# cvlab-dresden/DSAC

Measured on AMD Instinct MI355X. Metric: hypotheses scored/sec over 640x480 coord map, higher is better.
Workload: dtype f32

## Files before the change

dsac_amd/csrc/k2_plan.h:

```cpp
#pragma once

namespace dk {

struct K2Opts {
    bool pixel_minor = true;
    int flags = 0;
    int variant = -1;
    bool exact_auto = true;
    int diag = 0;
    int f16_store = 1;
};
enum { K2_ELEM_F32 = 0, K2_ELEM_F16 = 1, K2_ELEM_BF16 = 2 };
constexpr int K2_FLAG_STORE_ONLY = 1 << 1;
constexpr int K2_FLAG_ERR_UNFUSED = 1 << 24;
constexpr int K2_FLAG_PRECISE = 1 << 25;
constexpr int K2_FLAG_REC32 = 1 << 26;
constexpr int K2_FLAG_RECLO = 1 << 27;
constexpr int K2_FLAG_EXACT = 1 << 28;
constexpr int K2_FLAG_EXACT_ANY = 1 << 29;
enum { K2_FORM_NONE = 0, K2_FORM_FP32_VALU = 1, K2_FORM_FP32_MFMA = 2, K2_FORM_RECLO = 3, K2_FORM_EXACT_VEC = 4, K2_FORM_EXACT_ANY = 5, K2_FORM_PRECISE = 6 };
enum { K2_WHY_AUTO_OFF = 1, K2_WHY_FORCED = 2, K2_WHY_FOCAL = 4, K2_WHY_NO_POSES = 8 };
constexpr int K2_NF_MULTIPLE = 128;
constexpr int K2_WG = 256;

inline bool k2_wants_exact(const K2Opts& o) {
    if (o.flags & (K2_FLAG_EXACT | K2_FLAG_EXACT_ANY)) return true;
    return o.exact_auto && o.variant < 0 && !(o.flags & (K2_FLAG_PRECISE | K2_FLAG_RECLO | K2_FLAG_STORE_ONLY | K2_FLAG_REC32));
}

enum { K2_EXONLY_OK = 0, K2_EXONLY_VARIANT = 1, K2_EXONLY_FLAGS = 2, K2_EXONLY_AUTO_OFF = 3 };
inline int k2_exact_only(int variant, int flags, bool exact_auto) {
    const int ex_bits = K2_FLAG_EXACT | K2_FLAG_EXACT_ANY;
    if (variant != -1) return K2_EXONLY_VARIANT;
    if (flags & ~ex_bits) return K2_EXONLY_FLAGS;
    if (!exact_auto && !(flags & ex_bits)) return K2_EXONLY_AUTO_OFF;
    return K2_EXONLY_OK;
}

constexpr double K2_BIG_BYTES = 1.0e9, K2_HUGE_BYTES = 4.4e9;
inline double k2_err_bytes(int N, int P) { return (double)N * (double)P * 4.0; }
constexpr int K2_SMALL_MAP_CELLS = 16384;

inline bool k2_fuse_sums(const K2Opts& o, int N, int P, bool want_err, bool want_soft) {
    return !want_soft && want_err && o.variant < 0 && !(o.flags & K2_FLAG_ERR_UNFUSED) && k2_err_bytes(N, P) > K2_BIG_BYTES;
}

#define K2_FP32_IDS(VA, HP, ST, PS)                                                                                                                         \
    VA(0, 4, 32, false) VA(1, 4, 32, true) VA(2, 4, 16, false) VA(3, 4, 64, false) VA(10, 4, 1, false) VA(11, 4, 2, false) VA(12, 4, 4, false)               \
    VA(13, 4, 8, false)                                                                                                                                     \
    HP(20, 64, 2) HP(21, 64, 4) HP(22, 128, 2) HP(23, 32, 2) HP(24, 64, 1) HP(25, 128, 4) HP(26, 32, 4) HP(27, 128, 1)                                         \
    ST(40, 1, 1, 4, false, 1) ST(41, 2, 1, 4, false, 1) ST(42, 4, 1, 4, false, 1) ST(43, 2, 2, 4, false, 1)                                                   \
    ST(44, 1, 4, 1, true, 1) ST(45, 2, 4, 1, true, 1) ST(46, 4, 4, 1, true, 1) ST(47, 1, 2, 1, true, 1) ST(48, 2, 2, 1, true, 1) ST(49, 4, 2, 1, true, 1)       \
    ST(50, 1, 1, 1, true, 1) ST(51, 2, 1, 1, true, 1) ST(52, 4, 1, 1, true, 1) ST(53, 2, 1, 4, true, 1) ST(54, 2, 2, 4, true, 1) ST(55, 4, 1, 4, true, 1)       \
    ST(56, 2, 4, 4, true, 1) ST(57, 4, 2, 4, true, 1) ST(58, 4, 4, 1, true, 4) ST(59, 2, 4, 1, true, 5)                                                       \
    PS(60, 1) PS(61, 2) PS(62, 4)                                                                                                                           \
    ST(65, 4, 4, 4, true, 4) ST(66, 4, 4, 2, true, 4) ST(67, 1, 4, 4, true, 1) ST(68, 2, 4, 4, false, 1) ST(69, 2, 4, 8, true, 1) ST(70, 2, 4, 4, true, 4)     \
    ST(71, 1, 4, 8, true, 1) ST(72, 2, 4, 16, true, 1) ST(73, 2, 8, 1, true, 1) ST(74, 1, 8, 1, true, 1) ST(75, 2, 6, 1, true, 1) ST(76, 2, 3, 1, true, 1)     \
    ST(77, 1, 6, 1, true, 1)                                                                                                                                \
    ST(80, 4, 4, 1, true, 4) ST(81, 4, 4, 1, true, 4) ST(82, 4, 4, 1, true, 4) ST(83, 4, 4, 1, true, 4) ST(84, 4, 4, 1, true, 4) ST(85, 4, 4, 1, true, 4)     \
    ST(89, 4, 4, 1, true, 4) ST(93, 4, 4, 1, true, 4) ST(94, 4, 4, 1, true, 4) ST(95, 4, 4, 1, true, 4)
#define K2_RECLO_IDS(LO) LO(80, 4, 4, 3) LO(81, 4, 4, 2) LO(82, 4, 2, 4) LO(83, 2, 4, 3)
constexpr int K2_RECLO_DEFAULT_ID = 81;
#define K2_EXACT_IDS(EX) EX(84, 4, 4, 2, 1) EX(85, 4, 4, 2, 2) EX(89, 2, 4, 2, 1) EX(93, 4, 1, 3, 1) EX(94, 4, 1, 3, 2) EX(95, 4, 1, 4, 2)
#define K2_EXACT_AUTO_TILES(AX) AX(4, 1, 3) AX(4, 4, 2)

enum { K2_FAM_NONE = 0, K2_FAM_VALU_SCALAR, K2_FAM_VALU, K2_FAM_HP, K2_FAM_ST, K2_FAM_PS, K2_FAM_RECLO, K2_FAM_EXACT_VEC, K2_FAM_EXACT_ANY, K2_FAM_PRECISE };

struct K2Kernel {
    int family = K2_FAM_NONE, id = -1;
    int px = 0, ht = 0, ng = 0, ch = 0, wv = 0, pw = 0, minw = 0, exf = 0;
};
inline K2Kernel k2_fp32_kernel(int id) {
    K2Kernel k;
    switch (id) {
#define K2_VA_(ID, PX, HT, SP) case ID: k.family = K2_FAM_VALU; k.id = ID; k.px = PX; k.ht = HT; break;
#define K2_HP_(ID, HT, CH) case ID: k.family = K2_FAM_HP; k.id = ID; k.ht = HT; k.ch = CH; break;
#define K2_ST_(ID, NG, CH, WV, PW, MW) case ID: k.family = K2_FAM_ST; k.id = ID; k.ng = NG; k.ch = CH; k.wv = WV; k.pw = PW; k.minw = MW; break;
#define K2_PS_(ID, NG) case ID: k.family = K2_FAM_PS; k.id = ID; k.ng = NG; k.wv = 4; break;
        K2_FP32_IDS(K2_VA_, K2_HP_, K2_ST_, K2_PS_)
#undef K2_VA_
#undef K2_HP_
#undef K2_ST_
#undef K2_PS_
        default: break;
    }
    return k;
}
inline K2Kernel k2_reclo_kernel(int id) {
    K2Kernel k;
    switch (id) {
#define K2_LO_(ID, NG, CH, MW) case ID: k.family = K2_FAM_RECLO; k.id = ID; k.ng = NG; k.ch = CH; k.wv = 1; k.pw = 1; k.minw = MW; break;
        K2_RECLO_IDS(K2_LO_)
#undef K2_LO_
        default: break;
    }
    return k;
}
inline K2Kernel k2_exact_kernel(int id) {
    K2Kernel k;
    switch (id) {
#define K2_EX_(ID, NG, CH, MW, F) case ID: k.family = K2_FAM_EXACT_VEC; k.id = ID; k.ng = NG; k.ch = CH; k.wv = 1; k.pw = 1; k.minw = MW; k.exf = F; break;
        K2_EXACT_IDS(K2_EX_)
#undef K2_EX_
        default: break;
    }
    return k;
}
inline bool k2_variant_known(int v) { return v == -1 || k2_fp32_kernel(v).family != K2_FAM_NONE; }

inline int reproject_num_pixel_tiles(int P) { return (P + 63) / 64 + 15; }
inline int k2_ceil_div(int a, int b) { return (a + b - 1) / b; }
inline int k2_tiles(const K2Kernel& k, int P, bool soft) {
    switch (k.family) {
        case K2_FAM_VALU_SCALAR: return k2_ceil_div(P, K2_WG);
        case K2_FAM_VALU: return k2_ceil_div(P, K2_WG * k.px);
        case K2_FAM_HP: return k2_ceil_div(P, K2_WG * k.ch);
        case K2_FAM_PS: return k2_ceil_div(P, 64);
        case K2_FAM_PRECISE: return 2 * k2_ceil_div(P, K2_WG * 4);
        case K2_FAM_ST: case K2_FAM_RECLO: case K2_FAM_EXACT_VEC: case K2_FAM_EXACT_ANY: {
            const int PT = k2_ceil_div(P, k.wv * k.ch * 64);
            const int rows = k.pw ? PT * k.wv : PT;
            return rows + ((k.family == K2_FAM_EXACT_ANY && (P & 3) != 0 && soft) ? 1 : 0);
        }
        default: return 0;
    }
}

struct K2PlanIn {
    K2Opts o;
    int N = 0, Nf = 0, frames = 1;
    int P = 0, W = 0;
    bool uv = false;
    bool xyz_al16 = true, uv_al16 = true, err_al16 = true;
    bool focal_ok = true;
    bool poses = true;
    bool want_err = false, want_soft = false;
    int err_elem = K2_ELEM_F32;
};
constexpr int K2_STATUS_OK = 0, K2_STATUS_INVALID = 1, K2_STATUS_NOT_SUPPORTED = 801;
struct K2Plan {
    int status = K2_STATUS_OK;
    int form = K2_FORM_NONE, why = 0;
    K2Kernel k;
    bool need_split = false, need_lo = false;
    bool fuse_sums = false;
    int kflags = 0;
    bool pixel_minor = true;
    int Nf = 0;
    int tiles = 0;
};

inline K2Plan k2_plan(const K2PlanIn& in) {
    K2Plan p;
    const K2Opts& o = in.o;
    const bool fuse = k2_fuse_sums(o, in.N, in.P, in.want_err, in.want_soft);
    const bool err = in.want_err, soft = in.want_soft || fuse;
    if (in.N <= 0 || in.P <= 0 || (!err && !soft)) return p;
    auto refuse = [](int status) { K2Plan r; r.status = status; return r; };
    if (in.Nf <= 0 || in.frames <= 1) p.Nf = ((in.N + 127) / 128) * 128;
    else if (in.Nf % K2_NF_MULTIPLE != 0) return refuse(K2_STATUS_INVALID);
    else p.Nf = in.Nf;
    p.fuse_sums = fuse;
    const int variant = o.variant;
    const bool vec = in.P % 4 == 0 && in.err_al16 && in.xyz_al16 && in.uv_al16;
    p.kflags = o.flags | ((variant >= 40 && !o.pixel_minor) ? 32 : 0);
    p.pixel_minor = o.pixel_minor;
    const bool split_ok = in.poses && k2_wants_exact(o) && in.focal_ok;
    const K2Kernel exk = k2_exact_kernel(variant), lok = k2_reclo_kernel(variant);
    const bool ex_variant = exk.family != K2_FAM_NONE;
    int why = 0;
    if (!(o.flags & (K2_FLAG_EXACT | K2_FLAG_EXACT_ANY))) {
        if (variant >= 0 || (o.flags & (K2_FLAG_PRECISE | K2_FLAG_RECLO | K2_FLAG_STORE_ONLY | K2_FLAG_REC32))) why |= K2_WHY_FORCED;
        else if (!o.exact_auto) why |= K2_WHY_AUTO_OFF;
    } else if (variant >= 0 && !ex_variant) why |= K2_WHY_FORCED;
    if (!in.focal_ok) why |= K2_WHY_FOCAL;
    if (!in.poses) why |= K2_WHY_NO_POSES;
    if (in.err_elem != K2_ELEM_F32 && !(err && vec && in.P % 8 == 0 && split_ok && k2_exact_only(variant, o.flags, o.exact_auto) == K2_EXONLY_OK))
        return refuse(K2_STATUS_NOT_SUPPORTED);
    const bool prec_map = vec && (in.uv || in.W % 4 == 0);
    if (in.poses && (((o.flags & K2_FLAG_PRECISE) && !prec_map) || ((o.flags & K2_FLAG_RECLO) && !vec) || ((o.flags & K2_FLAG_EXACT) && !(vec && split_ok)) ||
                     ((o.flags & K2_FLAG_EXACT_ANY) && !(split_ok && (variant < 0 || (ex_variant && vec))))))
        return refuse(K2_STATUS_NOT_SUPPORTED);
    if ((o.flags & K2_FLAG_EXACT_ANY) && !in.poses) return refuse(K2_STATUS_NOT_SUPPORTED);
    const bool small_map = in.P <= K2_SMALL_MAP_CELLS;
    if ((o.flags & K2_FLAG_PRECISE) && in.poses && prec_map) {
        p.form = K2_FORM_PRECISE;
        p.k.family = K2_FAM_PRECISE;
// ... 44 lines not shown
```

dsac_amd/csrc/k_forward.hip:

```cpp
#include "kernels.h"
#include <hip/hip_ext.h>
#include "dmath.h"

namespace dk {

typedef float f4 __attribute__((ext_vector_type(4)));
typedef float f2 __attribute__((ext_vector_type(2)));
typedef _Float16 h4 __attribute__((ext_vector_type(4)));

DM_INLINE void pose_focal(const float4* __restrict__ cams, int h, int Nf, float& fx, float& fy) {
    if (!cams) return;
    const float4 k = cams[Nf > 0 ? h / Nf : 0];
    fx = k.x; fy = k.y;
}
DM_INLINE int split_exponent_of(float fx, float fy) {
    int e = 0;
    while (e < 31 && (float)(1u << e) < fmaxf(fx, fy)) e++;
    return e;
}
__global__ __launch_bounds__(256) void k_pose_prep(int N, const double* __restrict__ poses, float fx, float fy, float* __restrict__ staged,
                                                   const float4* __restrict__ cams, int Nf) {
    const int h = blockIdx.x * blockDim.x + threadIdx.x;
    if (h >= N) return;
    pose_focal(cams, h, Nf, fx, fy);
// ... 455 lines not shown
    if (pt >= PT) return;
    const int h0 = ht * HT;
    const int nh = min(HT, N - h0);
    const int tid = threadIdx.x, lane = tid & 63, wave = tid >> 6;
    const int c = lane & 15, g = lane >> 4;
    {
        const int frame = h0 / Nf;
        xyz += (long long)frame * xyz_stride;
        if (UV) uv += (long long)frame * uv_stride;
    }

    __shared__ float s_A[(HT / 16) * 3 * 64];
    __shared__ float s_soft[SOFT ? (K2_THREADS / 64) * HT : 1];
    for (int i = tid; i < (HT / 16) * 3 * 64; i += K2_THREADS) {
        const int l = i & 63, cg = i >> 6;
        const int comp = cg % 3, gi = cg / 3;
        const int hyp = min(16 * gi + (l & 15), nh - 1), k = l >> 4;
        const float v = staged[(size_t)(h0 + hyp) * POSE_STRIDE + comp * 4 + k];
        s_A[i] = comp < 2 ? -v : v;
    }

    float Bm[KM_CH][4];
    f2 ppix[KM_CH][4];
    int p0[KM_CH];
    bool valid[KM_CH];
#pragma unroll
    for (int ch = 0; ch < KM_CH; ch++) {
        const int chunk0 = (pt * (K2_THREADS / 64) * KM_CH + wave * KM_CH + ch) * 64;
        p0[ch] = chunk0 + 4 * c;
        valid[ch] = p0[ch] < P;
#pragma unroll
        for (int m = 0; m < 4; m++) {
            const int pc = min(p0[ch] + m, P - 1);
            Bm[ch][m] = (g < 3) ? xyz[(size_t)pc * 3 + g] : 1.0f;
        }
        if (UV) {
            if (valid[ch]) {
                const f4* su = reinterpret_cast<const f4*>(uv + (size_t)p0[ch] * 2);
                const f4 u0 = su[0], u1 = su[1];
                ppix[ch][0] = f2{u0.x - cx, u0.y - cy}; ppix[ch][1] = f2{u0.z - cx, u0.w - cy};
                ppix[ch][2] = f2{u1.x - cx, u1.y - cy}; ppix[ch][3] = f2{u1.z - cx, u1.w - cy};
            } else {
                ppix[ch][0] = ppix[ch][1] = ppix[ch][2] = ppix[ch][3] = splat(0.f);
            }
        } else {
            int y = p0[ch] / W, x = p0[ch] - y * W;
#pragma unroll
            for (int m = 0; m < 4; m++) {
                ppix[ch][m] = f2{(float)x - cx, (float)y - cy};
                if (++x == W) { x = 0; y++; }
            }
        }
    }
    __syncthreads();

    for (int gi = 0; gi < HT / 16; gi++) {
        if (16 * gi >= nh) break;
        const float ax = s_A[(gi * 3 + 0) * 64 + lane], ay = s_A[(gi * 3 + 1) * 64 + lane], az = s_A[(gi * 3 + 2) * 64 + lane];
        const int hyp0 = 16 * gi + 4 * g;
        f2 ssum[4] = {splat(0.f), splat(0.f), splat(0.f), splat(0.f)};
#pragma unroll
        for (int ch = 0; ch < KM_CH; ch++) {
            f4 ev[4];
            f2 sloc[4];
            if (kflags & 2) {
                if (ERR && valid[ch]) {
                    f4* dst = reinterpret_cast<f4*>(err + (size_t)(h0 + hyp0) * P + p0[ch]);
                    const size_t rs = (size_t)P / 4;
                    const f4 o = {ax, ay, az, (float)gi};
#pragma unroll
                    for (int r = 0; r < 4; r++) {
                        if (hyp0 + r >= nh) continue;
                        f4* q = dst + r * rs;
                        const int mode = (kflags >> 2) & 7;
                        if (mode == 0) __builtin_nontemporal_store(o, q);
                        else if (mode == 1) *q = o;
                        else if (mode == 2) asm volatile("global_store_dwordx4 %0, %1, off sc1" ::"v"(q), "v"(o) : "memory");
                        else if (mode == 3) asm volatile("global_store_dwordx4 %0, %1, off sc0 sc1" ::"v"(q), "v"(o) : "memory");
                        else if (mode == 4) asm volatile("global_store_dwordx4 %0, %1, off sc1 nt" ::"v"(q), "v"(o) : "memory");
                        else asm volatile("global_store_dwordx4 %0, %1, off sc0" ::"v"(q), "v"(o) : "memory");
                    }
                }
                continue;
            }
            if (__builtin_expect(__any(hp_chunk<false, SOFT>(ax, ay, az, Bm[ch], ppix[ch], clampv, kA, kB, ev, sloc)), 0))
                (void)hp_chunk<true, SOFT>(ax, ay, az, Bm[ch], ppix[ch], clampv, kA, kB, ev, sloc);
            if (SOFT) {
                const f2 vf = splat(valid[ch] ? 1.0f : 0.0f);
#pragma unroll
                for (int r = 0; r < 4; r++) ssum[r] = pk_fma(sloc[r], vf, ssum[r]);
            }
            if (ERR && valid[ch]) {
                f4* dst = reinterpret_cast<f4*>(err + (size_t)(h0 + hyp0) * P + p0[ch]);
                const size_t rs = (size_t)P / 4;
                if (nh == HT) {
#pragma unroll
                    for (int r = 0; r < 4; r++) {
                        if (kflags & 1) dst[r * rs] = ev[r]; else __builtin_nontemporal_store(ev[r], dst + r * rs);
                    }
                } else {
#pragma unroll
                    for (int r = 0; r < 4; r++) {
                        if (hyp0 + r < nh) { if (kflags & 1) dst[r * rs] = ev[r]; else __builtin_nontemporal_store(ev[r], dst + r * rs); }
                    }
                }
            }
        }
        if (SOFT) {
            const float s0 = row16_sum(ssum[0].x + ssum[0].y), s1 = row16_sum(ssum[1].x + ssum[1].y);
            const float s2 = row16_sum(ssum[2].x + ssum[2].y), s3 = row16_sum(ssum[3].x + ssum[3].y);
            if (c == 0) {
                float* dst = s_soft + wave * HT + hyp0;
                if (hyp0 + 0 < nh) dst[0] = s0;
                if (hyp0 + 1 < nh) dst[1] = s1;
                if (hyp0 + 2 < nh) dst[2] = s2;
                if (hyp0 + 3 < nh) dst[3] = s3;
            }
        }
    }

    if (SOFT) {
        __syncthreads();
        if (tid < nh) {
            float s = 0.f;
#pragma unroll
            for (int w = 0; w < K2_THREADS / 64; w++) s += s_soft[w * HT + tid];
            soft_part[(size_t)pt * N + h0 + tid] = s;
        }
    }
}

template <int HT, int KM_CH>
static hipError_t launch_reproject_hp(hipStream_t st, int N, const float* staged, const FrameDev& F, float clampv, float* err, float kA,
                                      float kB, float* soft_part, int Nf, bool pixel_minor, int kflags, hipEvent_t evA, hipEvent_t evB) {
    const int tile = K2_THREADS * KM_CH;
    const int PT = (F.P + tile - 1) / tile;
    const int NTa = (N + HT - 1) / HT;
    const int grid = ((PT + 7) / 8) * 8 * NTa;
    const int NT = pixel_minor ? -NTa : NTa;
    const bool ERR = err != nullptr, SOFT = soft_part != nullptr, UV = F.uv != nullptr;
    const size_t lds_pad = (size_t)((kflags >> 8) & 0xff) * 8192;
#define DSAC_K2H(E, S, U)                                                                                                             \
    hipExtLaunchKernelGGL((k_reproject_hp<HT, E, S, U, KM_CH>), dim3(grid), dim3(K2_THREADS), lds_pad, st, evA, evB, 0, staged, F.xyz, F.uv, err,   \
                          soft_part, N, F.P, F.W, PT, NT, F.cx, F.cy, clampv, kA, kB, kflags, Nf, F.xyz_stride, F.uv_stride)
    if (ERR && SOFT) { if (UV) DSAC_K2H(true, true, true); else DSAC_K2H(true, true, false); }
    else if (ERR) { if (UV) DSAC_K2H(true, false, true); else DSAC_K2H(true, false, false); }
    else if (SOFT) { if (UV) DSAC_K2H(false, true, true); else DSAC_K2H(false, true, false); }
#undef DSAC_K2H
    return hipGetLastError();
}

typedef f4 f4_a4 __attribute__((aligned(4)));
typedef unsigned u2v __attribute__((ext_vector_type(2)));
template <int LAYOUT, bool BF = false>
DM_INLINE void store_rows_h16(_Float16* base, const f4 (&ev)[4], int P, int p0, int g, int c, bool full, int rows) {
    const __amdgpu_buffer_rsrc_t rsrc = __builtin_amdgcn_make_buffer_rsrc(base, 0, 0xffffffffu, 0x00020000);
    unsigned pk[4][2];
#pragma unroll
    for (int r = 0; r < 4; r++) { pk[r][0] = pk_e2<BF>(ev[r].x, ev[r].y); pk[r][1] = pk_e2<BF>(ev[r].z, ev[r].w); }
    if constexpr (LAYOUT == 1) {
        const unsigned loff = ((unsigned)(4 * g) * (unsigned)P + (unsigned)p0) * 2u;
        if (full) {
#pragma unroll
            for (int r = 0; r < 4; r++) __builtin_amdgcn_raw_buffer_store_b64(u2v{pk[r][0], pk[r][1]}, rsrc, loff, (unsigned)r * (unsigned)P * 2u, 2);
        } else {
#pragma unroll
            for (int r = 0; r < 4; r++)
                if (r < rows) __builtin_amdgcn_raw_buffer_store_b64(u2v{pk[r][0], pk[r][1]}, rsrc, loff, (unsigned)r * (unsigned)P * 2u, 2);
        }
    } else {
        const bool odd = (c & 1) != 0;
        auto nb = [](unsigned v) { return (unsigned)__builtin_amdgcn_update_dpp(0, (int)v, 0xB1, 0xf, 0xf, true); };
        unsigned nk[4][2];
#pragma unroll
        for (int r = 0; r < 4; r++) { nk[r][0] = nb(pk[r][0]); nk[r][1] = nb(pk[r][1]); }
        const u4v ra = {odd ? nk[2][0] : pk[0][0], odd ? nk[2][1] : pk[0][1], odd ? pk[2][0] : nk[0][0], odd ? pk[2][1] : nk[0][1]};
        const u4v rb = {odd ? nk[3][0] : pk[1][0], odd ? nk[3][1] : pk[1][1], odd ? pk[3][0] : nk[1][0], odd ? pk[3][1] : nk[1][1]};
        const int r0 = odd ? 2 : 0;
        const unsigned loff = ((unsigned)(4 * g + r0) * (unsigned)P + (unsigned)(p0 & ~7)) * 2u;
        if (full) {
            __builtin_amdgcn_raw_buffer_store_b128(ra, rsrc, loff, 0u, 2);
            __builtin_amdgcn_raw_buffer_store_b128(rb, rsrc, loff, (unsigned)P * 2u, 2);
        } else {
            if (r0 < rows) __builtin_amdgcn_raw_buffer_store_b128(ra, rsrc, loff, 0u, 2);
            if (r0 + 1 < rows) __builtin_amdgcn_raw_buffer_store_b128(rb, rsrc, loff, (unsigned)P * 2u, 2);
        }
    }
}
template <int NG, int CHW, int WAVES, bool PW, bool ERR, bool SOFT, bool UV, bool G64, int MINW, bool LO = false, int EXF = 0, int ANY = 0>
__global__ __launch_bounds__(WAVES * 64, MINW) void k_reproject_st(const float* __restrict__ staged, const float* __restrict__ xyz,
                                                             const float* __restrict__ uv, float* __restrict__ err,
                                                             float* __restrict__ soft_part, int N, int P, int W, int PT, float cx, float cy,
                                                             float clampv, float kA, float kB, int kflags, int Nf, long long xyz_stride,
                                                             long long uv_stride, const float* __restrict__ staged_lo = nullptr,
                                                             const void* __restrict__ split = nullptr, const float4* __restrict__ cams = nullptr) {
    constexpr int HT = 16 * NG;
    constexpr bool EX = EXF != 0, RSQ = EXF >= 2;
    constexpr bool BF16 = EXF >= 5;
    constexpr int H16 = EXF >= 5 ? EXF - 4 : EXF >= 3 ? EXF - 2 : 0;
    static_assert(H16 == 0 || (ERR && ANY == 0 && !LO), "half error images: the vector build of the exact form, with an error image to store");
    const int b = blockIdx.x;
    int ht, pt;
    if (kflags & 32) { pt = b % PT; ht = b / PT; }
    else if (WAVES == 1) {
        const int q = b >> 5, sub = (b >> 3) & 3, PTG = (PT + 31) >> 5;
        ht = q / PTG;
        pt = ((q % PTG) * 8 + (b & 7)) * 4 + sub;
        if (pt >= PT) return;
    } else {
        const int q = b >> 3, PTG = (PT + 7) >> 3;
        ht = q / PTG;
        pt = (q % PTG) * 8 + (b & 7);
        if (pt >= PT) return;
    }
    const int h0 = ht * HT;
    const int nh = min(HT, N - h0);
    const int tid = threadIdx.x, lane = tid & 63;
    const int wave = __builtin_amdgcn_readfirstlane(tid >> 6);
    const int c = lane & 15, g = lane >> 4;
    {
        const int frame = h0 / Nf;
        xyz += (long long)frame * xyz_stride;
        if (UV) uv += (long long)frame * uv_stride;
        if (EX && cams) {
            const float4 k = cams[frame];
            cx = k.z; cy = k.w;
        }
    }
    __shared__ float s_soft[(SOFT && !PW) ? WAVES * HT : 1];

    float Bm[CHW][4];
    f2 ppix[G64 ? 1 : CHW][4];
    int sx0[G64 ? CHW : 1];
    float sby[G64 ? CHW : 1];
    int p0[CHW];
    bool valid[CHW];
    const int chunk0 = (pt * WAVES + wave) * CHW + (ANY == 2 ? (P - 1) >> 6 : 0);
#pragma unroll
    for (int ch = 0; ch < CHW; ch++) {
        p0[ch] = (chunk0 + ch) * 64 + 4 * c;
        if constexpr (ANY == 1) valid[ch] = p0[ch] + 3 < P;
        else if constexpr (ANY == 2) valid[ch] = p0[ch] < P && p0[ch] + 3 >= P;
        else valid[ch] = p0[ch] < P;
#pragma unroll
        for (int m = 0; m < 4; m++) {
            const int pc = min(p0[ch] + m, P - 1);
            Bm[ch][m] = (g < 3) ? xyz[(size_t)pc * 3 + g] : 1.0f;
        }
    }
    h8 B8[EX ? CHW : 1][4];
    bool oor[EX ? CHW : 1];
    if (EX) {
#pragma unroll
        for (int ch = 0; ch < CHW; ch++) {
            bool o = false;
#pragma unroll
            for (int m = 0; m < 4; m++) B8[ch][m] = split_B((g < 3) ? Bm[ch][m] : SPLIT_T_COORD, o);
            oor[ch] = __any(o);
        }
    }
    h4 B16[LO ? CHW : 1][4];
    if (LO) {
#pragma unroll
        for (int ch = 0; ch < CHW; ch++)
#pragma unroll
            for (int m = 0; m < 4; m++) {
                const unsigned v = __builtin_bit_cast(unsigned, Bm[ch][m]);
                const auto r16 = __builtin_amdgcn_permlane16_swap(v, v, false, false);
                const auto r32 = __builtin_amdgcn_permlane32_swap(v, v, false, false);
                const unsigned u16 = r16[1], u32 = r32[1];
                const float s = 1.52587890625e-05f;
                const float X = Bm[ch][m] * s, Y = __builtin_bit_cast(float, u16) * s, Z = __builtin_bit_cast(float, u32) * s;
                const bool r0 = g == 0;
                B16[ch][m] = h4{(_Float16)(r0 ? X : 0.f), (_Float16)(r0 ? Y : 0.f), (_Float16)(r0 ? Z : 0.f), (_Float16)(r0 ? 0.00390625f : 0.f)};
            }
    }
    constexpr bool A_AHEAD = NG > 2;
    float ax[EX ? 1 : NG], ay[EX ? 1 : NG], az[EX ? 1 : NG];
    LoOps alo[LO ? NG : 1];
    ExOps aex[EX ? NG : 1];
    auto load_A = [&](int gi) {
        const int hyp = min(16 * gi + c, nh - 1);
        if (EX) {
            const h8* rc = reinterpret_cast<const h8*>(split) + (size_t)(h0 + hyp) * 12 + g;
            const h4* rh = reinterpret_cast<const h4*>(reinterpret_cast<const char*>(split) + (size_t)N * SPLIT_CROSS_BYTES) + (size_t)(h0 + hyp) * 12 + g;
            aex[gi].cx = rc[0]; aex[gi].cy = rc[4]; aex[gi].cz = rc[8];
            aex[gi].hx = rh[0]; aex[gi].hy = rh[4]; aex[gi].hz = rh[8];
            return;
        }
        const float* rec = staged + (size_t)(h0 + hyp) * POSE_STRIDE + g;
        ax[gi] = rec[0]; ay[gi] = rec[4]; az[gi] = rec[8];
        if (LO) {
            const f4* rl = reinterpret_cast<const f4*>(staged_lo + (size_t)(h0 + hyp) * POSE_STRIDE);
            const float S = (g == 0) ? 65536.f : 0.f, T = (g == 0) ? 256.f : 0.f;
            const f4 lx = rl[0], ly = rl[1], lz = rl[2];
            alo[gi].x = h4{(_Float16)(-lx.x * S), (_Float16)(-lx.y * S), (_Float16)(-lx.z * S), (_Float16)(-lx.w * T)};
            alo[gi].y = h4{(_Float16)(-ly.x * S), (_Float16)(-ly.y * S), (_Float16)(-ly.z * S), (_Float16)(-ly.w * T)};
            alo[gi].z = h4{(_Float16)(lz.x * S), (_Float16)(lz.y * S), (_Float16)(lz.z * S), (_Float16)(lz.w * T)};
        }
    };
#pragma unroll
    for (int gi = 0; gi < (A_AHEAD ? 1 : NG); gi++) load_A(gi);
#pragma unroll
    for (int ch = 0; ch < CHW; ch++) {
        if (UV) {
            constexpr int pc = G64 ? 0 : 1;
            if constexpr (ANY != 0) {
                if (valid[ch]) {
                    f4 u0, u1;
                    if constexpr (ANY != 2) {
                        const f4_a4* su = reinterpret_cast<const f4_a4*>(uv + (size_t)p0[ch] * 2);
                        u0 = su[0]; u1 = su[1];
                    } else {
                        const float* s1 = uv + (size_t)min(p0[ch] + 1, P - 1) * 2;
                        const float* s2 = uv + (size_t)min(p0[ch] + 2, P - 1) * 2;
                        const float* s3 = uv + (size_t)(P - 1) * 2;
                        u0 = f4{uv[(size_t)p0[ch] * 2], uv[(size_t)p0[ch] * 2 + 1], s1[0], s1[1]};
                        u1 = f4{s2[0], s2[1], s3[0], s3[1]};
                    }
                    ppix[ch * pc][0] = f2{u0.x - cx, u0.y - cy}; ppix[ch * pc][1] = f2{u0.z - cx, u0.w - cy};
                    ppix[ch * pc][2] = f2{u1.x - cx, u1.y - cy}; ppix[ch * pc][3] = f2{u1.z - cx, u1.w - cy};
                } else {
                    ppix[ch * pc][0] = ppix[ch * pc][1] = ppix[ch * pc][2] = ppix[ch * pc][3] = splat(0.f);
                }
            } else if (valid[ch]) {
                const f4* su = reinterpret_cast<const f4*>(uv + (size_t)p0[ch] * 2);
                const f4 u0 = su[0], u1 = su[1];
                ppix[ch * pc][0] = f2{u0.x - cx, u0.y - cy}; ppix[ch * pc][1] = f2{u0.z - cx, u0.w - cy};
                ppix[ch * pc][2] = f2{u1.x - cx, u1.y - cy}; ppix[ch * pc][3] = f2{u1.z - cx, u1.w - cy};
            } else {
                ppix[ch * pc][0] = ppix[ch * pc][1] = ppix[ch * pc][2] = ppix[ch * pc][3] = splat(0.f);
            }
        } else if (G64) {
            const int cpr = W >> 6;
            const int y = (chunk0 + ch) / cpr, xc0 = ((chunk0 + ch) - y * cpr) * 64;
            sx0[ch] = __builtin_amdgcn_readfirstlane(xc0);
            sby[ch] = __builtin_bit_cast(float, __builtin_amdgcn_readfirstlane(__builtin_bit_cast(int, (float)y - cy)));
        } else {
            constexpr int pc = G64 ? 0 : 1;
            int y = p0[ch] / W, x = p0[ch] - y * W;
#pragma unroll
            for (int m = 0; m < 4; m++) {
                ppix[ch * pc][m] = f2{(float)x - cx, (float)y - cy};
                if (++x == W) { x = 0; y++; }
            }
        }
    }

#pragma unroll
    for (int gi = 0; gi < NG; gi++) {
        if (16 * gi >= nh) break;
        if (A_AHEAD && gi + 1 < NG) {
            asm volatile("" ::: "memory");
            load_A(gi + 1);
        }
        const float nax = EX ? 0.f : -ax[EX ? 0 : gi], nay = EX ? 0.f : -ay[EX ? 0 : gi];
        const int hyp0 = 16 * gi + 4 * g;
        bool grp_far = false;
        if constexpr (ANY != 0 && EX) grp_far = __any((float)aex[gi].hx[3] != 0.f || (float)aex[gi].hy[3] != 0.f || (float)aex[gi].hz[3] != 0.f);
        f2 ssum[4] = {splat(0.f), splat(0.f), splat(0.f), splat(0.f)};
#pragma unroll
        for (int ch = 0; ch < CHW; ch++) {
            f4 ev[4];
            f2 sloc[4];
            if (G64) {
                f2 pb = f2{(float)(sx0[ch] + 4 * c) - cx, sby[ch]};
                asm volatile("" : "+v"(pb));
#pragma unroll
                for (int m = 0; m < 4; m++) ppix[0][m] = f2{pb.x + (float)m, pb.y};
            }
            const f2 (&pp)[4] = ppix[G64 ? 0 : ch];
            if (EX) {
                if (__builtin_expect(oor[ch] || grp_far, 0)) {
                    const int hyp = min(16 * gi + c, nh - 1);
                    const float* rec = staged + (size_t)(h0 + hyp) * POSE_STRIDE + g;
                    float Bf[4];
#pragma unroll
                    for (int m = 0; m < 4; m++) Bf[m] = (g < 3) ? xyz[(size_t)min(p0[ch] + m, P - 1) * 3 + g] : 1.0f;
                    (void)hp_chunk<true, SOFT, false>(-rec[0], -rec[4], rec[8], Bf, pp, clampv, kA, kB, ev, sloc);
                } else if (__builtin_expect(__any(hp_chunk_ex<false, SOFT, RSQ>(aex[gi], B8[ch], pp, clampv, kA, kB, ev, sloc)), 0)) {
                    (void)hp_chunk_ex<true, SOFT>(aex[gi], B8[ch], pp, clampv, kA, kB, ev, sloc);
                }
            } else if (kflags & 2) {
                ev[0] = ev[1] = ev[2] = ev[3] = f4{nax, nay, az[EX ? 0 : gi], (float)ch};
                sloc[0] = sloc[1] = sloc[2] = sloc[3] = splat(0.f);
            } else if (__builtin_expect(__any(hp_chunk<false, SOFT, LO>(nax, nay, az[EX ? 0 : gi], Bm[ch], pp, clampv, kA, kB, ev, sloc, &alo[LO ? gi : 0], B16[LO ? ch : 0])), 0)) {
                (void)hp_chunk<true, SOFT, LO>(nax, nay, az[EX ? 0 : gi], Bm[ch], pp, clampv, kA, kB, ev, sloc, &alo[LO ? gi : 0], B16[LO ? ch : 0]);
            }
            if constexpr (ANY == 2) {
                const int nv = P - p0[ch];
                if (SOFT) {
                    const f2 m01 = {nv > 0 ? 1.0f : 0.0f, nv > 1 ? 1.0f : 0.0f}, m23 = {nv > 2 ? 1.0f : 0.0f, nv > 3 ? 1.0f : 0.0f};
#pragma unroll
                    for (int r = 0; r < 4; r++)
                        sloc[r] = pk_fma(soft_inlier2(f2{ev[r].x, ev[r].y}, kA, kB), m01, soft_inlier2(f2{ev[r].z, ev[r].w}, kA, kB) * m23);
                }
            }
            if (SOFT) {
                const f2 vf = splat(valid[ch] ? 1.0f : 0.0f);
#pragma unroll
                for (int r = 0; r < 4; r++) ssum[r] = pk_fma(sloc[r], vf, ssum[r]);
            }
            bool fast_stores = true;
            if constexpr (ANY != 0) {
                fast_stores = ANY == 1;
                if (ERR && valid[ch] && !fast_stores) {
                    const int nv = P - p0[ch];
                    const __amdgpu_buffer_rsrc_t rsrc = __builtin_amdgcn_make_buffer_rsrc(err + (size_t)(h0 + 16 * gi) * P, 0, 0xffffffffu, 0x00020000);
                    const unsigned loff = ((unsigned)(4 * g) * (unsigned)P + (unsigned)p0[ch]) * 4u;
#pragma unroll
                    for (int r = 0; r < 4; r++) {
                        if (hyp0 + r >= nh) continue;
                        const unsigned soff = (unsigned)r * (unsigned)P * 4u;
                        const float ex = ev[r].x, ey = ev[r].y, ez = ev[r].z, ew = ev[r].w;
                        __builtin_amdgcn_raw_buffer_store_b32(__float_as_uint(ex), rsrc, loff, soff, 2);
                        if (nv > 1) __builtin_amdgcn_raw_buffer_store_b32(__float_as_uint(ey), rsrc, loff + 4u, soff, 2);
                        if (nv > 2) __builtin_amdgcn_raw_buffer_store_b32(__float_as_uint(ez), rsrc, loff + 8u, soff, 2);
                        if (nv > 3) __builtin_amdgcn_raw_buffer_store_b32(__float_as_uint(ew), rsrc, loff + 12u, soff, 2);
                    }
                }
            }
            if constexpr (H16 != 0) {
                if (valid[ch]) store_rows_h16<H16, BF16>(reinterpret_cast<_Float16*>(err) + (size_t)(h0 + 16 * gi) * P, ev, P, p0[ch], g, c, nh == HT, nh - hyp0);
            }
            if (H16 == 0 && ERR && valid[ch] && fast_stores) {
                const __amdgpu_buffer_rsrc_t rsrc = __builtin_amdgcn_make_buffer_rsrc(err + (size_t)(h0 + 16 * gi) * P, 0, 0xffffffffu, 0x00020000);
                const unsigned loff = ((unsigned)(4 * g) * (unsigned)P + (unsigned)p0[ch]) * 4u;
                if (nh == HT) {
#pragma unroll
                    for (int r = 0; r < 4; r++) __builtin_amdgcn_raw_buffer_store_b128(__builtin_bit_cast(u4v, ev[r]), rsrc, loff, (unsigned)r * (unsigned)P * 4u, 2);
                } else {
#pragma unroll
                    for (int r = 0; r < 4; r++)
                        if (hyp0 + r < nh) __builtin_amdgcn_raw_buffer_store_b128(__builtin_bit_cast(u4v, ev[r]), rsrc, loff, (unsigned)r * (unsigned)P * 4u, 2);
                }
            }
            if (ERR && !SOFT) {
                const int ps = (kflags >> 16) & 15, pn = (kflags >> 20) & 15;
                for (int i = 0; i < ps; i++) __builtin_amdgcn_s_sleep(1);
                for (int i = 0; i < pn; i++) asm volatile("s_nop 15");
            }
        }
        if (SOFT) {
            const float s0 = row16_sum(ssum[0].x + ssum[0].y), s1 = row16_sum(ssum[1].x + ssum[1].y);
            const float s2 = row16_sum(ssum[2].x + ssum[2].y), s3 = row16_sum(ssum[3].x + ssum[3].y);
            if (c == 0) {
                float* dst = !PW ? s_soft + wave * HT + hyp0 : soft_part + (size_t)(pt * WAVES + wave) * N + h0 + hyp0;
                if (hyp0 + 0 < nh) dst[0] = s0;
                if (hyp0 + 1 < nh) dst[1] = s1;
                if (hyp0 + 2 < nh) dst[2] = s2;
                if (hyp0 + 3 < nh) dst[3] = s3;
            }
        }
    }
    if (SOFT && !PW) {
        __syncthreads();
        if (tid < nh) {
            float s = 0.f;
#pragma unroll
            for (int w = 0; w < WAVES; w++) s += s_soft[w * HT + tid];
            soft_part[(size_t)pt * N + h0 + tid] = s;
        }
    }
}

template <int NG>
struct K2Ops {
    float B[4];
    float A[NG][3];
};

template <int NG, int WAVES, bool ERR, bool SOFT, bool UV>
__global__ __launch_bounds__(WAVES * 64) void k_reproject_ps(const float* __restrict__ staged, const float* __restrict__ xyz,
                                                             const float* __restrict__ uv, float* __restrict__ err,
                                                             float* __restrict__ soft_part, int N, int P, int W, float cx, float cy,
                                                             float clampv, float kA, float kB, int kflags, int Nf, long long xyz_stride,
                                                             long long uv_stride) {
    constexpr int HT = 16 * NG;
    const int tid = threadIdx.x, lane = tid & 63;
    const int wave = __builtin_amdgcn_readfirstlane(tid >> 6);
    const int c = lane & 15, g = lane >> 4;
    const int xcd = blockIdx.x & 7, lwg = blockIdx.x >> 3, GX = gridDim.x >> 3;
    const int CR = (P + 63) >> 6;
    const int UR = (CR + WAVES - 1) / WAVES;
    const int URX = (UR + 7) >> 3;
    const int NRG = (N + HT - 1) / HT;
    const int TT = NRG * URX;

    auto decode = [&](int tw, int& h0, int& chunk) {
        const int rg = tw / URX, ux = tw - rg * URX;
        const int unit = ux * 8 + xcd;
        h0 = rg * HT;
        chunk = (tw < TT && unit < UR) ? unit * WAVES + wave : -1;
        if (chunk >= CR) chunk = -1;
    };
    auto issue = [&](int tw, K2Ops<NG>& o) {
        int h0, chunk;
        decode(min(tw, TT - 1), h0, chunk);
// ... 577 lines not shown
```

Measured before the change: 3.880 million.

## Add specialized interior fast path with explicit vmcnt waits and fenced error stores

Adds a dedicated loop for full interior tiles of the exact-form kernel (no out-of-range chunks, full hypothesis group, G64 layout, no UV). It waits on vector memory counters with explicit immediates so the prefetch of the next group's pose data can overlap outstanding error-image stores. It also groups the stores with scheduling barriers and a short nop. A new flag can force the original general path. The extra waits and fences may serialize more than the compiler would on its own, and the added variant increases code size.

Measured after the change: 3.973 million (median of 6 runs). +2.4%, better.

```diff
diff --git a/dsac_amd/csrc/k2_plan.h b/dsac_amd/csrc/k2_plan.h
--- a/dsac_amd/csrc/k2_plan.h
+++ b/dsac_amd/csrc/k2_plan.h
@@ -18,6 +18,7 @@
 constexpr int K2_FLAG_RECLO = 1 << 27;
 constexpr int K2_FLAG_EXACT = 1 << 28;
 constexpr int K2_FLAG_EXACT_ANY = 1 << 29;
+constexpr int K2_FLAG_GENERAL_PATH = 1 << 30;
 enum { K2_FORM_NONE = 0, K2_FORM_FP32_VALU = 1, K2_FORM_FP32_MFMA = 2, K2_FORM_RECLO = 3, K2_FORM_EXACT_VEC = 4, K2_FORM_EXACT_ANY = 5, K2_FORM_PRECISE = 6 };
 enum { K2_WHY_AUTO_OFF = 1, K2_WHY_FORCED = 2, K2_WHY_FOCAL = 4, K2_WHY_NO_POSES = 8 };
 constexpr int K2_NF_MULTIPLE = 128;
@@ -32,7 +33,7 @@
 inline int k2_exact_only(int variant, int flags, bool exact_auto) {
     const int ex_bits = K2_FLAG_EXACT | K2_FLAG_EXACT_ANY;
     if (variant != -1) return K2_EXONLY_VARIANT;
-    if (flags & ~ex_bits) return K2_EXONLY_FLAGS;
+    if (flags & ~(ex_bits | K2_FLAG_GENERAL_PATH)) return K2_EXONLY_FLAGS;
     if (!exact_auto && !(flags & ex_bits)) return K2_EXONLY_AUTO_OFF;
     return K2_EXONLY_OK;
 }
diff --git a/dsac_amd/csrc/k_forward.hip b/dsac_amd/csrc/k_forward.hip
--- a/dsac_amd/csrc/k_forward.hip
+++ b/dsac_amd/csrc/k_forward.hip
@@ -631,7 +631,13 @@
 
 typedef f4 f4_a4 __attribute__((aligned(4)));
 typedef unsigned u2v __attribute__((ext_vector_type(2)));
-template <int LAYOUT, bool BF = false>
+DM_INLINE void k2_stores_begin() { __builtin_amdgcn_sched_barrier(0); }
+DM_INLINE void k2_stores_end() {
+    __builtin_amdgcn_sched_barrier(0);
+    asm volatile("s_nop 3");
+    __builtin_amdgcn_sched_barrier(0);
+}
+template <int LAYOUT, bool BF = false, bool FENCE = false>
 DM_INLINE void store_rows_h16(_Float16* base, const f4 (&ev)[4], int P, int p0, int g, int c, bool full, int rows) {
     const __amdgpu_buffer_rsrc_t rsrc = __builtin_amdgcn_make_buffer_rsrc(base, 0, 0xffffffffu, 0x00020000);
     unsigned pk[4][2];
@@ -640,8 +646,10 @@
     if constexpr (LAYOUT == 1) {
         const unsigned loff = ((unsigned)(4 * g) * (unsigned)P + (unsigned)p0) * 2u;
         if (full) {
+            if (FENCE) k2_stores_begin();
 #pragma unroll
             for (int r = 0; r < 4; r++) __builtin_amdgcn_raw_buffer_store_b64(u2v{pk[r][0], pk[r][1]}, rsrc, loff, (unsigned)r * (unsigned)P * 2u, 2);
+            if (FENCE) k2_stores_end();
         } else {
 #pragma unroll
             for (int r = 0; r < 4; r++)
@@ -658,14 +666,17 @@
         const int r0 = odd ? 2 : 0;
         const unsigned loff = ((unsigned)(4 * g + r0) * (unsigned)P + (unsigned)(p0 & ~7)) * 2u;
         if (full) {
+            if (FENCE) k2_stores_begin();
             __builtin_amdgcn_raw_buffer_store_b128(ra, rsrc, loff, 0u, 2);
             __builtin_amdgcn_raw_buffer_store_b128(rb, rsrc, loff, (unsigned)P * 2u, 2);
+            if (FENCE) k2_stores_end();
         } else {
             if (r0 < rows) __builtin_amdgcn_raw_buffer_store_b128(ra, rsrc, loff, 0u, 2);
             if (r0 + 1 < rows) __builtin_amdgcn_raw_buffer_store_b128(rb, rsrc, loff, (unsigned)P * 2u, 2);
         }
     }
 }
+constexpr int k2_vmcnt_imm(int n) { return (n & 15) | ((n >> 4) << 14) | 0x0f70; }
 template <int NG, int CHW, int WAVES, bool PW, bool ERR, bool SOFT, bool UV, bool G64, int MINW, bool LO = false, int EXF = 0, int ANY = 0>
 __global__ __launch_bounds__(WAVES * 64, MINW) void k_reproject_st(const float* __restrict__ staged, const float* __restrict__ xyz,
                                                              const float* __restrict__ uv, float* __restrict__ err,
@@ -823,6 +834,70 @@
                 ppix[ch * pc][m] = f2{(float)x - cx, (float)y - cy};
                 if (++x == W) { x = 0; y++; }
             }
+        }
+    }
+
+    if constexpr (EXF >= 2 && ANY == 0 && !LO && G64 && !UV && PW && MINW <= 3) {
+        bool far = false;
+#pragma unroll
+        for (int ch = 0; ch < CHW; ch++) far = far || oor[ch];
+        if (nh == HT && (chunk0 + CHW) * 64 <= P && !far && !(kflags & K2_FLAG_GENERAL_PATH)) {
+            constexpr int GRP_STORES = ERR ? CHW * (H16 == 2 ? 2 : 4) : 0;
+            __builtin_amdgcn_s_waitcnt(k2_vmcnt_imm(0));
+#pragma unroll
+            for (int gi = 0; gi < NG; gi++) {
+                if (A_AHEAD && gi > 0) {
+                    __builtin_amdgcn_s_waitcnt(k2_vmcnt_imm(GRP_STORES));
+                    asm volatile("" : "+v"(aex[gi].cx), "+v"(aex[gi].cy), "+v"(aex[gi].cz), "+v"(aex[gi].hx), "+v"(aex[gi].hy), "+v"(aex[gi].hz));
+                }
+                if (A_AHEAD && gi + 1 < NG) {
+                    asm volatile("" ::: "memory");
+                    load_A(gi + 1);
+                }
+                const int hyp0 = 16 * gi + 4 * g;
+                f2 ssum[4] = {splat(0.f), splat(0.f), splat(0.f), splat(0.f)};
+#pragma unroll
+                for (int ch = 0; ch < CHW; ch++) {
+                    f4 ev[4];
+                    f2 sloc[4];
+                    f2 pb = f2{(float)(sx0[ch] + 4 * c) - cx, sby[ch]};
+                    asm volatile("" : "+v"(pb));
+#pragma unroll
+                    for (int m = 0; m < 4; m++) ppix[0][m] = f2{pb.x + (float)m, pb.y};
+                    if (__builtin_expect(__any(hp_chunk_ex<false, SOFT, RSQ>(aex[gi], B8[ch], ppix[0], clampv, kA, kB, ev, sloc)), 0)) {
+                        (void)hp_chunk_ex<true, SOFT>(aex[gi], B8[ch], ppix[0], clampv, kA, kB, ev, sloc);
+                    }
+                    if (SOFT) {
+                        const f2 vf = splat(1.0f);
+#pragma unroll
+                        for (int r = 0; r < 4; r++) ssum[r] = pk_fma(sloc[r], vf, ssum[r]);
+                    }
+                    if constexpr (H16 != 0) {
+                        store_rows_h16<H16, BF16, true>(reinterpret_cast<_Float16*>(err) + (size_t)(h0 + 16 * gi) * P, ev, P, p0[ch], g, c, true, 4);
+                    } else if (ERR) {
+                        const __amdgpu_buffer_rsrc_t rsrc = __builtin_amdgcn_make_buffer_rsrc(err + (size_t)(h0 + 16 * gi) * P, 0, 0xffffffffu, 0x00020000);
+                        const unsigned loff = ((unsigned)(4 * g) * (unsigned)P + (unsigned)p0[ch]) * 4u;
+                        k2_stores_begin();
+#pragma unroll
+                        for (int r = 0; r < 4; r++) __builtin_amdgcn_raw_buffer_store_b128(__builtin_bit_cast(u4v, ev[r]), rsrc, loff, (unsigned)r * (unsigned)P * 4u, 2);
+                        k2_stores_end();
+                    }
+                    if (ERR && !SOFT) {
+                        const int ps = (kflags >> 16) & 15, pn = (kflags >> 20) & 15;
+                        for (int i = 0; i < ps; i++) __builtin_amdgcn_s_sleep(1);
+                        for (int i = 0; i < pn; i++) asm volatile("s_nop 15");
+                    }
+                }
+                if (SOFT) {
+                    const float s0 = row16_sum(ssum[0].x + ssum[0].y), s1 = row16_sum(ssum[1].x + ssum[1].y);
+                    const float s2 = row16_sum(ssum[2].x + ssum[2].y), s3 = row16_sum(ssum[3].x + ssum[3].y);
+                    if (c == 0) {
+                        float* dst = soft_part + (size_t)(pt * WAVES + wave) * N + h0 + hyp0;
+                        dst[0] = s0; dst[1] = s1; dst[2] = s2; dst[3] = s3;
+                    }
+                }
+            }
+            return;
         }
     }
 
```
